# Jordy-VL/multi-modal-early-exit

Measured on AMD Instinct MI355X. Metric: docs_per_sec, higher is better.
Workload: dtype f32 (operands split into 2 x f16, 3 f16 MFMA terms per MAC, f32 accumulate)

## Files before the change

multi-modal-early-exit_amd/csrc/gemm_split.hip:

```cpp
#include <cstdlib>
#include "mmee_common.h"

#include "gemm_split_kernel.h"

namespace mmee {

bool gemm_split_supports(int N, int K) { return N > 0 && K > 0 && N % 256 == 0 && K % 32 == 0; }

void launch_split_ffn_up(const GemmArgs& a, int max_m, int num_cus, hipStream_t s);

void launch_gemm_split(const GemmArgs& a_in, int epi, int max_m, int num_cus, hipStream_t s) {
    GemmArgs a = a_in;
    a.tile_order = a.N <= 768 ? 1 : 0;
    if (a.probe) a.terms = 3;
    if (a.probe) {
        if (a.out_split && epi == EPI_GELU) { launch_split_one<CfgP, EPI_GELU, true, false, 1>(a, max_m, num_cus, s); return; }
        if (!a.out_split && epi == EPI_RESID) { launch_split_one<CfgP, EPI_RESID, false, false, 1>(a, max_m, num_cus, s); return; }
        if (!a.out_split && epi == EPI_BIAS) { launch_split_one<CfgP, EPI_BIAS, false, false, 1>(a, max_m, num_cus, s); return; }
        if (!a.out_split && epi == EPI_TANH) { launch_split_one<CfgP, EPI_TANH, false, false, 1>(a, max_m, num_cus, s); return; }
    }
    if (a.k_splits > 1 && !a.out_split && epi == EPI_BIAS && a.terms != 1) {
        a.tile_counter = nullptr;
        launch_split_one<CfgP, EPI_BIAS, false, false, 1>(a, max_m, num_cus, s);
        return;
    }
    a.k_splits = 1;
    if (a.terms != 1 && (long)((max_m + 255) / 256) * (a.N / 256) * 2 <= (long)num_cus) {
        a.tile_counter = nullptr;
        if (a.out_split && epi == EPI_GELU) { launch_split_one<CfgP, EPI_GELU, true, false, 1>(a, max_m, num_cus, s); return; }
        if (a.out_split && epi == EPI_BIAS) { launch_split_one<CfgP, EPI_BIAS, true, false, 1>(a, max_m, num_cus, s); return; }
        if (!a.out_split && epi == EPI_RESID) { launch_split_one<CfgP, EPI_RESID, false, false, 1>(a, max_m, num_cus, s); return; }
        if (!a.out_split && epi == EPI_BIAS) { launch_split_one<CfgP, EPI_BIAS, false, false, 1>(a, max_m, num_cus, s); return; }
        if (!a.out_split && epi == EPI_TANH) { launch_split_one<CfgP, EPI_TANH, false, false, 1>(a, max_m, num_cus, s); return; }
        a.tile_counter = a_in.tile_counter;
    }
#ifdef MMEE_DIAG
    static const int order_env = diag_env_int("MMEE_GEMM_ORDER", -1);
    if (order_env == 0 || order_env == 1) a.tile_order = order_env;
    else if (order_env == 2) a.tile_order = a.N <= 768 ? 1 : 0;
    else if (order_env == 3 || order_env == 4) a.tile_order = a.N >= 2304 ? order_env - 1 : a.tile_order;
    static const int forced = diag_env_int("MMEE_SPLIT_CFG", 0);
    const bool use_a = forced == 1;
    if (a.dbg_noload && (forced == 0 || forced == 3)) {
        if (a.out_split && epi == EPI_GELU) launch_split_one<CfgC, EPI_GELU, true, true>(a, max_m, num_cus, s);
        else if (a.out_split) launch_split_one<CfgC, EPI_BIAS, true, true>(a, max_m, num_cus, s);
        else launch_split_one<CfgC, EPI_RESID, false, true>(a, max_m, num_cus, s);
        return;
    }
    if (a.dbg_noload) {
        if (a.out_split) launch_split_one<CfgA, EPI_GELU, true, true>(a, max_m, num_cus, s);
        else if (use_a) launch_split_one<CfgA, EPI_RESID, false, true>(a, max_m, num_cus, s);
        else launch_split_one<CfgB, EPI_RESID, false, true>(a, max_m, num_cus, s);
        return;
    }
    if (forced == 1 || forced == 2) {
        if (a.out_split) {
            if (epi == EPI_GELU && use_a) launch_split_one<CfgA, EPI_GELU, true>(a, max_m, num_cus, s);
            else if (epi == EPI_GELU) launch_split_one<CfgB, EPI_GELU, true>(a, max_m, num_cus, s);
            else if (use_a) launch_split_one<CfgA, EPI_BIAS, true>(a, max_m, num_cus, s);
            else launch_split_one<CfgB, EPI_BIAS, true>(a, max_m, num_cus, s);
            return;
        }
        if (use_a) {
            switch (epi) {
                case EPI_BIAS: launch_split_one<CfgA, EPI_BIAS, false>(a, max_m, num_cus, s); break;
                case EPI_GELU: launch_split_one<CfgA, EPI_GELU, false>(a, max_m, num_cus, s); break;
                case EPI_RESID: launch_split_one<CfgA, EPI_RESID, false>(a, max_m, num_cus, s); break;
                default: launch_split_one<CfgA, EPI_TANH, false>(a, max_m, num_cus, s); break;
            }
            return;
        }
        switch (epi) {
            case EPI_BIAS: launch_split_one<CfgB, EPI_BIAS, false>(a, max_m, num_cus, s); break;
            case EPI_GELU: launch_split_one<CfgB, EPI_GELU, false>(a, max_m, num_cus, s); break;
            case EPI_RESID: launch_split_one<CfgB, EPI_RESID, false>(a, max_m, num_cus, s); break;
            default: launch_split_one<CfgB, EPI_TANH, false>(a, max_m, num_cus, s); break;
        }
        return;
    }
#endif
    if (a.terms == 1) {
        if (a.out_split && epi == EPI_GELU) { launch_split_one<CfgC, EPI_GELU, true, false, 0, 1>(a, max_m, num_cus, s); return; }
        if (a.out_split && epi == EPI_BIAS) { launch_split_one<CfgC, EPI_BIAS, true, false, 0, 1>(a, max_m, num_cus, s); return; }
        if (!a.out_split && epi == EPI_RESID) {
            if (a.role_tag == 3) launch_split_one<CfgC, EPI_RESID, false, false, 3, 1>(a, max_m, num_cus, s);
            else launch_split_one<CfgC, EPI_RESID, false, false, 2, 1>(a, max_m, num_cus, s);
            return;
        }
    }
    if (a.out_split) {
        if (epi == EPI_GELU) launch_split_ffn_up(a, max_m, num_cus, s);
        else launch_split_one<CfgC, EPI_BIAS, true>(a, max_m, num_cus, s);
        return;
    }
    switch (epi) {
        case EPI_BIAS: launch_split_one<CfgC, EPI_BIAS, false>(a, max_m, num_cus, s); break;
        case EPI_GELU: launch_split_one<CfgC, EPI_GELU, false>(a, max_m, num_cus, s); break;
        case EPI_RESID:
            if (a.role_tag == 2) launch_split_one<CfgC, EPI_RESID, false, false, 2>(a, max_m, num_cus, s);
            else if (a.role_tag == 3) launch_split_one<CfgC, EPI_RESID, false, false, 3>(a, max_m, num_cus, s);
            else launch_split_one<CfgC, EPI_RESID, false>(a, max_m, num_cus, s);
            break;
        default: launch_split_one<CfgC, EPI_TANH, false>(a, max_m, num_cus, s); break;
    }
}

__global__ __launch_bounds__(256) void split_rows_kernel(const float* __restrict__ src, char* __restrict__ dst, const int* __restrict__ n_rows_ptr,
                                                         int n_rows_static, int K, float scale, int* __restrict__ err_flag) {
    const int n_rows = n_rows_ptr ? *n_rows_ptr : n_rows_static;
    const int k4 = K / 4;
    const size_t total = (size_t)n_rows * k4;
    float amax = 0.f;
    for (size_t i = (size_t)blockIdx.x * 256 + threadIdx.x; i < total; i += (size_t)gridDim.x * 256) {
        const size_t r = i / k4;
        const int c = (int)(i - r * k4) * 4;
        const f32x4 v = *reinterpret_cast<const f32x4*>(src + r * K + c);
        store_split4(dst + r * (size_t)K * 4, c, v, scale, amax);
    }
    split_flag_overflow(amax, err_flag);
}

void launch_split_rows(const float* src, void* dst, const int* n_rows_ptr, int n_rows_static, int max_rows, int K, float scale, int num_cus,
                       hipStream_t s, int* err_flag) {
    size_t total = (size_t)max_rows * (K / 4);
    size_t blocks = (total + 255) / 256;
    int grid = (int)(blocks < (size_t)num_cus * 16 ? blocks : (size_t)num_cus * 16);
    if (grid < 1) grid = 1;
    hipLaunchKernelGGL(split_rows_kernel, dim3(grid), dim3(256), 0, s, src, reinterpret_cast<char*>(dst), n_rows_ptr, n_rows_static, K, scale, err_flag);
}

__global__ __launch_bounds__(256) void patch_split_kernel(const float* __restrict__ pix, char* __restrict__ dst, int n_patches, int C, int R,
                                                          int P, int G, float scale, int* __restrict__ err_flag) {
    const int K = C * P * P, k4 = K / 4;
    const size_t total = (size_t)n_patches * k4;
    float amax = 0.f;
    for (size_t i = (size_t)blockIdx.x * 256 + threadIdx.x; i < total; i += (size_t)gridDim.x * 256) {
        const size_t r = i / k4;
        const int k = (int)(i - r * k4) * 4;
        const int b = (int)(r / (size_t)(G * G)), pr = (int)(r - (size_t)b * (G * G));
        const int gy = pr / G, gx = pr - gy * G;
        const int c = k / (P * P), rem = k - c * P * P;
        const int py = rem / P, px = rem - py * P;
        const f32x4 v = *reinterpret_cast<const f32x4*>(pix + (((size_t)b * C + c) * R + (size_t)(gy * P + py)) * R + gx * P + px);
        store_split4_quad(dst + r * (size_t)K * 4, k, v, scale, amax, threadIdx.x & 63);
    }
    split_flag_overflow(amax, err_flag);
}

void launch_patch_split(const float* pix, void* dst, int n_docs, int C, int R, int P, float scale, int num_cus, hipStream_t s, int* err_flag) {
    const int G = R / P;
    const size_t total = (size_t)n_docs * G * G * (C * P * P / 4);
    size_t blocks = (total + 255) / 256;
    int grid = (int)(blocks < (size_t)num_cus * 16 ? blocks : (size_t)num_cus * 16);
    if (grid < 1) grid = 1;
    hipLaunchKernelGGL(patch_split_kernel, dim3(grid), dim3(256), 0, s, pix, reinterpret_cast<char*>(dst), n_docs * G * G, C, R, P, G, scale, err_flag);
}

__global__ __launch_bounds__(256) void absmax_kernel(const float* __restrict__ src, size_t n, float* __restrict__ out) {
    float m = 0.f;
    for (size_t i = (size_t)blockIdx.x * 256 + threadIdx.x; i < n; i += (size_t)gridDim.x * 256) m = fmaxf(m, fabsf(src[i]));
    m = wave_max(m);
    if ((threadIdx.x & 63) == 0) atomicMax(reinterpret_cast<unsigned*>(out), __float_as_uint(m));
}

void launch_absmax(const float* src, size_t n, float* out_dev, hipStream_t s) {
    (void)hipMemsetAsync(out_dev, 0, sizeof(float), s);
    size_t blocks = (n + 255) / 256;
    int grid = (int)(blocks < 1024 ? blocks : 1024);
    if (grid < 1) grid = 1;
    hipLaunchKernelGGL(absmax_kernel, dim3(grid), dim3(256), 0, s, src, n, out_dev);
}

}
```

multi-modal-early-exit_amd/csrc/gemm_split_ffn_up.hip:

```cpp
#include "gemm_split_kernel.h"

namespace mmee {

void launch_split_ffn_up(const GemmArgs& a, int max_m, int num_cus, hipStream_t s) {
    launch_split_one<CfgC, EPI_GELU, true>(a, max_m, num_cus, s);
}

}
```

multi-modal-early-exit_amd/csrc/gemm_split_kernel.h:

```cpp
#pragma once
#include <cstdlib>
#include "mmee_common.h"

namespace mmee {


template <int BM_, int BN_, int ROWB_, int NST_, int WM_, int WN_, int WGS_, int MF_ = 32>
struct SplitCfg {
    static constexpr int BM = BM_, BN = BN_, ROWB = ROWB_, NST = NST_, WM = WM_, WN = WN_, WGS = WGS_;
    static constexpr int MF = MF_;
    static_assert(MF == 32 || (MF == 16 && ROWB == 128), "the 16x16x32 MFMA consumes one 128-byte row (k = 32) per step");
    static constexpr int NW = WM * WN, THREADS = NW * 64;
    static constexpr int KSTAGE = ROWB / 4;
    static constexpr int PROWS = 1024 / ROWB;
    static constexpr int PA = BM / PROWS / NW, PW = BN / PROWS / NW;
    static constexpr int PP = PA + PW;
    static constexpr int A_BYTES = BM * ROWB, STAGE_BYTES = (BM + BN) * ROWB, LOOP_BYTES = NST * STAGE_BYTES;
    static constexpr int EPI_BYTES = NW * 32 * 64 * 4;
    static_assert(BM == WM * 64 && BN == WN * 64, "one 64x64 sub-tile per wave");
    static_assert(PA * PROWS * NW == BM && PW * PROWS * NW == BN && PA >= 1 && PW >= 1, "DMA pieces must tile the stage");
    static_assert(EPI_BYTES <= LOOP_BYTES, "epilogue staging must fit in the stage ring");
    static_assert(NST >= 2 && NST <= 4, "ring depth");
    static_assert(THREADS <= 1024, "a workgroup is at most 16 waves");
    static_assert(WGS * (LOOP_BYTES + 16) <= 160 * 1024, "LDS budget of a CU (160 KiB) for WGS workgroups");
    static_assert(WGS * NW <= 32, "wave slots of a CU");
};
using CfgA = SplitCfg<128, 256, 64, 3, 2, 4, 2>;
using CfgB = SplitCfg<256, 256, 128, 2, 4, 4, 1>;
using CfgC = SplitCfg<256, 256, 128, 2, 4, 4, 1, 16>;
using CfgP = SplitCfg<128, 128, 128, 3, 2, 2, 1, 16>;


__device__ __forceinline__ void dma_piece(unsigned voff, unsigned long long base, unsigned lds_addr) {
    unsigned keep;
    asm volatile("s_mov_b32 %0, m0\n\ts_mov_b32 m0, %2\n\ts_nop 0\n\tglobal_load_lds_dwordx4 %1, %3\n\ts_mov_b32 m0, %0"
                 : "=&s"(keep)
                 : "v"(voff), "s"(lds_addr), "s"(base)
                 : "memory");
}

template <int EPI, bool OUT_SPLIT, int WN>
__device__ __forceinline__ void split_store_tile(const GemmArgs& g, float* smem, f32x16 (&acc)[2][2], int m0, int n0, int M,
                                                 int wave, int lane) {
    const int wr = wave / WN, wc = wave % WN;
    const int l31 = lane & 31, hh = lane >> 5;
    float* stg = smem + wave * (32 * 64);
    const int c4 = (lane & 15) * 4;
    const int col = n0 + wc * 64 + c4;
    f32x4 bv = f32x4{0.f, 0.f, 0.f, 0.f};
    if (g.bias) bv = *reinterpret_cast<const f32x4*>(g.bias + col);
    const float sc = (col < g.scale_cols) ? g.scale : 1.0f;
    f32x4 lam = f32x4{1.f, 1.f, 1.f, 1.f};
    if (g.col_scale) lam = *reinterpret_cast<const f32x4*>(g.col_scale + col);
    const float alpha = g.alpha;
    float amax = 0.f;
#pragma unroll
    for (int mi = 0; mi < 2; ++mi) {
#pragma unroll
        for (int ni = 0; ni < 2; ++ni)
#pragma unroll
            for (int e = 0; e < 16; ++e) {
                const int r = (e & 3) + 8 * (e >> 2) + 4 * hh;
                stg[r * 64 + ni * 32 + l31] = acc[mi][ni][e];
            }
        asm volatile("" ::: "memory");
        const int rbase = m0 + wr * 64 + mi * 32 + (lane >> 4);
#pragma unroll 4
        for (int j = 0; j < 8; ++j) {
            const int rl = (lane >> 4) + 4 * j;
            const int row = rbase + 4 * j;
            f32x4 v = *reinterpret_cast<const f32x4*>(stg + rl * 64 + c4);
            if (row < M) {
#pragma unroll
                for (int t = 0; t < 4; t += 2) {
                    f32x2 x = __builtin_elementwise_fma(f32x2{v[t], v[t + 1]}, (f32x2)(alpha), f32x2{bv[t], bv[t + 1]}) * (f32x2)(sc);
                    if (EPI == EPI_GELU) x = gelu_erf2(x);
                    if (EPI == EPI_TANH) { x[0] = tanhf(x[0]); x[1] = tanhf(x[1]); }
                    x = x * f32x2{lam[t], lam[t + 1]};
                    v[t] = x[0];
                    v[t + 1] = x[1];
                }
                if (EPI == EPI_RESID) {
                    const int rs = g.resid_row_src ? g.resid_row_src[row] : row;
                    if (g.resid_split_inv != 0.f) {
                        const f32x4 r = load_split4_sum(g.resid + (size_t)rs * g.ldr, col);
#pragma unroll
                        for (int t = 0; t < 4; t += 2) {
                            const f32x2 y = __builtin_elementwise_fma(f32x2{r[t], r[t + 1]}, (f32x2)(g.resid_split_inv), f32x2{v[t], v[t + 1]});
                            v[t] = y[0];
                            v[t + 1] = y[1];
                        }
                    } else {
                        v += *reinterpret_cast<const f32x4*>(g.resid + (size_t)rs * g.ldr + col);
                    }
                }
                if (!OUT_SPLIT) *reinterpret_cast<f32x4*>(g.C + (size_t)row * g.ldc + col) = v;
            }
            if (OUT_SPLIT) {
                f16x4 hi, lo;
                split_f16x4(row < M ? v : f32x4{0.f, 0.f, 0.f, 0.f}, g.out_scale, hi, lo, amax);
                const int2 h2 = __builtin_bit_cast(int2, hi), l2 = __builtin_bit_cast(int2, lo);
                const bool take_lo = (lane & 2) != 0;
                int4 piece;
                {
                    const int a0 = __builtin_amdgcn_mov_dpp(h2.x, 0x88, 0xf, 0xf, true), a1 = __builtin_amdgcn_mov_dpp(h2.y, 0x88, 0xf, 0xf, true);
                    const int b0 = __builtin_amdgcn_mov_dpp(l2.x, 0x88, 0xf, 0xf, true), b1 = __builtin_amdgcn_mov_dpp(l2.y, 0x88, 0xf, 0xf, true);
                    const int c0 = __builtin_amdgcn_mov_dpp(h2.x, 0xDD, 0xf, 0xf, true), c1 = __builtin_amdgcn_mov_dpp(h2.y, 0xDD, 0xf, 0xf, true);
                    const int d0 = __builtin_amdgcn_mov_dpp(l2.x, 0xDD, 0xf, 0xf, true), d1 = __builtin_amdgcn_mov_dpp(l2.y, 0xDD, 0xf, 0xf, true);
                    piece.x = take_lo ? b0 : a0;
                    piece.y = take_lo ? b1 : a1;
                    piece.z = take_lo ? d0 : c0;
                    piece.w = take_lo ? d1 : c1;
                }
                if (row < M)
                    *reinterpret_cast<int4*>(reinterpret_cast<char*>(g.C) + (size_t)row * g.ldc * 4 + (size_t)(col >> 4) * 64 + (lane & 3) * 16) = piece;
            }
        }
    }
    if (OUT_SPLIT) split_flag_overflow(amax, g.err_flag);
}

template <int EPI, bool OUT_SPLIT, int WN, int RB>
__device__ __forceinline__ void split_store_tile16(const GemmArgs& g, float* smem, f32x4 (&acc)[4][4], int m0, int n0, int M,
                                                   int wave, int lane, const f32x4 bv, const f32x4 lam, const size_t c_shift = 0) {
    const int wr = wave / WN, wc = wave % WN;
    const int l15 = lane & 15, gq = lane >> 4;
    float* stg = smem + wave * (RB * 64);
    const int c4 = (lane & 15) * 4;
    const int col = n0 + wc * 64 + c4;
    const float sc = (col < g.scale_cols) ? g.scale : 1.0f;
    const float s_out = OUT_SPLIT ? g.out_scale : 1.0f;
    constexpr bool ACT = EPI == EPI_GELU || EPI == EPI_TANH;
    const bool sc_p2 = (__float_as_uint(sc) & 0x007fffffu) == 0u;
    const float fold = ACT ? 1.0f : s_out * (sc_p2 ? sc : 1.0f);
    const float post = ACT ? sc : (sc_p2 ? 1.0f : sc);
    const bool need_post = __builtin_amdgcn_readfirstlane((int)__float_as_uint(post)) != 0x3f800000;
    const bool need_lam = g.col_scale != nullptr;
    const float alpha_e = g.alpha * fold;
    const f32x4 be = bv * fold;
    const float gelu_c0 = __builtin_log2f(s_out) - 1.0f, gelu_hs = 0.5f * s_out;
    float amax = 0.f;
#pragma unroll
    for (int half = 0; half < 64 / RB; ++half) {
#pragma unroll
        for (int m2 = 0; m2 < RB / 16; ++m2)
#pragma unroll
            for (int ni = 0; ni < 4; ++ni)
#pragma unroll
                for (int e = 0; e < 4; ++e) {
                    const int r = 16 * m2 + 4 * gq + e;
                    stg[r * 64 + ((ni * 16 + l15) ^ (16 * (gq & 1)))] = acc[(RB / 16) * half + m2][ni][e];
                }
        asm volatile("" ::: "memory");
        const int rbase = m0 + wr * 64 + half * RB + (lane >> 4);
#pragma unroll
        for (int j = 0; j < RB / 4; ++j) {
            const int rl = (lane >> 4) + 4 * j;
            const int row = rbase + 4 * j;
            f32x4 v = *reinterpret_cast<const f32x4*>(stg + rl * 64 + (c4 ^ (16 * ((rl >> 2) & 1))));
#pragma unroll
            for (int t = 0; t < 4; t += 2) {
                f32x2 x = __builtin_elementwise_fma(f32x2{v[t], v[t + 1]}, (f32x2)(alpha_e), f32x2{be[t], be[t + 1]});
                if (need_post) x = x * (f32x2)(post);
                if (EPI == EPI_GELU) x = gelu_scaled2(x, gelu_c0, gelu_hs);
                if (EPI == EPI_TANH) { x[0] = tanhf(x[0]) * s_out; x[1] = tanhf(x[1]) * s_out; }
                if (need_lam) x = x * f32x2{lam[t], lam[t + 1]};
                v[t] = x[0];
                v[t + 1] = x[1];
            }
            if (row < M) {
                if (EPI == EPI_RESID) {
                    const int rs = g.resid_row_src ? g.resid_row_src[row] : row;
                    if (g.resid_split_inv != 0.f) {
                        const f32x4 r = load_split4_sum(g.resid + (size_t)rs * g.ldr, col);
#pragma unroll
                        for (int t = 0; t < 4; t += 2) {
                            const f32x2 y = __builtin_elementwise_fma(f32x2{r[t], r[t + 1]}, (f32x2)(g.resid_split_inv), f32x2{v[t], v[t + 1]});
                            v[t] = y[0];
                            v[t + 1] = y[1];
                        }
                    } else {
                        v += *reinterpret_cast<const f32x4*>(g.resid + (size_t)rs * g.ldr + col);
                    }
                }
                if (!OUT_SPLIT) *reinterpret_cast<f32x4*>(g.C + c_shift + (size_t)row * g.ldc + col) = v;
            }
            if (OUT_SPLIT) {
                int2 h2, l2;
                {
                    unsigned h01, h23, l01, l23;
                    split_pair(v[0], v[1], h01, l01, amax);
                    split_pair(v[2], v[3], h23, l23, amax);
                    h2.x = (int)h01; h2.y = (int)h23; l2.x = (int)l01; l2.y = (int)l23;
                }
                const bool take_lo = (lane & 2) != 0;
                int4 piece;
                {
                    const int a0 = __builtin_amdgcn_mov_dpp(h2.x, 0x88, 0xf, 0xf, true), a1 = __builtin_amdgcn_mov_dpp(h2.y, 0x88, 0xf, 0xf, true);
                    const int b0 = __builtin_amdgcn_mov_dpp(l2.x, 0x88, 0xf, 0xf, true), b1 = __builtin_amdgcn_mov_dpp(l2.y, 0x88, 0xf, 0xf, true);
                    const int c0 = __builtin_amdgcn_mov_dpp(h2.x, 0xDD, 0xf, 0xf, true), c1 = __builtin_amdgcn_mov_dpp(h2.y, 0xDD, 0xf, 0xf, true);
                    const int d0 = __builtin_amdgcn_mov_dpp(l2.x, 0xDD, 0xf, 0xf, true), d1 = __builtin_amdgcn_mov_dpp(l2.y, 0xDD, 0xf, 0xf, true);
                    piece.x = take_lo ? b0 : a0;
                    piece.y = take_lo ? b1 : a1;
                    piece.z = take_lo ? d0 : c0;
                    piece.w = take_lo ? d1 : c1;
                }
                if (row < M)
                    *reinterpret_cast<int4*>(reinterpret_cast<char*>(g.C) + (size_t)row * g.ldc * 4 + (size_t)(col >> 4) * 64 + (lane & 3) * 16) = piece;
            }
        }
        asm volatile("" ::: "memory");
    }
    if (OUT_SPLIT) split_flag_overflow(amax, g.err_flag);
}

template <typename Cfg, int EPI, bool OUT_SPLIT, bool DIAG = false, int TAG = 0, int TERMS = 3>
__global__ __launch_bounds__(Cfg::THREADS, 4) void gemm_split_kernel(const GemmArgs g) {
    constexpr int BM = Cfg::BM, BN = Cfg::BN, ROWB = Cfg::ROWB, NST = Cfg::NST, WN = Cfg::WN, PA = Cfg::PA, PW = Cfg::PW;
    constexpr int STAGE_BYTES = Cfg::STAGE_BYTES, A_BYTES = Cfg::A_BYTES;
    const int dbg = DIAG ? g.dbg_noload : 0;
    extern __shared__ __attribute__((aligned(16))) float smem[];
    const int M = g.m_ptr ? *g.m_ptr : g.m_static;
    const int tiles_m = (M + BM - 1) / BM;
    const int tiles_n = g.N / BN;
    constexpr bool KSPLIT = TAG == 1;
    const int ksp = KSPLIT && g.k_splits > 1 ? g.k_splits : 1;
    const int n_tiles = tiles_m * tiles_n * ksp;
    const int nk = g.K / Cfg::KSTAGE / ksp;
    int ks_pop = 0;
    const int tid = threadIdx.x;
    const int lane = tid & 63, wave = __builtin_amdgcn_readfirstlane(tid >> 6);
    const int wr = wave / WN, wc = wave % WN;
    const int l31 = lane & 31, hh = lane >> 5;

    unsigned long long clk0 = 0, rt0 = 0;
    if (DIAG && g.clk_probe) { clk0 = __builtin_amdgcn_s_memtime(); rt0 = __builtin_amdgcn_s_memrealtime(); }
    constexpr int GM = 8;
    int* q_slot = reinterpret_cast<int*>(reinterpret_cast<char*>(smem) + Cfg::LOOP_BYTES);
    const int n_groups = (tiles_m + GM - 1) / GM;
    const int my_xcd = g.tile_counter ? (int)(__builtin_amdgcn_s_getreg((3 << 11) | (0 << 6) | 20) & 7u) : 0;
    int q_try = 0;
    int tile = blockIdx.x;

    const unsigned lds0 = (unsigned)(size_t)(__attribute__((address_space(3))) float*)smem;
    constexpr int CPR = ROWB / 16;
    const int p_row = lane / CPR, p_chunk = lane % CPR;
    const int swz_even = ROWB == 64 ? ((p_row >> 2) & 3) : ((p_row >> 1) & 7);
    const unsigned chunk_even = 16u * (unsigned)(p_chunk ^ swz_even);
    const unsigned chunk_odd = ROWB == 64 ? chunk_even : 16u * (unsigned)(p_chunk ^ ((swz_even + 4) & 7));
    const unsigned rswz = ROWB == 64 ? (unsigned)((l31 >> 2) & 3) : (unsigned)((l31 >> 1) & 7);
    const unsigned a_row = (unsigned)(wr * 64 + l31) * ROWB;
    const unsigned w_row = (unsigned)A_BYTES + (unsigned)(wc * 64 + l31) * ROWB;
    const int l15 = lane & 15, lq = lane >> 4;
    const unsigned swz16 = (unsigned)((l15 >> 1) & 7);
    const unsigned c16_hi = 16u * (((unsigned)(lq & 1) + 4u * (unsigned)(lq >> 1)) ^ swz16);
    const unsigned c16_lo = 16u * (((unsigned)(lq & 1) + 4u * (unsigned)(lq >> 1) + 2u) ^ swz16);
    const unsigned a_row16 = (unsigned)(wr * 64 + l15) * ROWB;
    const unsigned w_row16 = (unsigned)A_BYTES + (unsigned)(wc * 64 + l15) * ROWB;
    const char* sbytes = reinterpret_cast<const char*>(smem);

    constexpr bool HANDOVER = Cfg::MF == 16 && NST == 2 && Cfg::NW * 4096 <= STAGE_BYTES;

    auto pop = [&](int& tm, int& tn) __attribute__((always_inline)) -> bool {
        if (g.tile_counter) {
            while (q_try < 8) {
                const int q = (my_xcd + q_try) & 7;
                if (tid == 0) *q_slot = atomicAdd(g.tile_counter + 16 * q, 1);
                __syncthreads();
                const int j = *q_slot;
                __syncthreads();
                if (g.tile_order >= 2) {
                    const int gq = q < n_groups ? (n_groups - q + 7) / 8 : 0;
                    if (g.tile_order == 2) {
                        constexpr int CW = 4;
                        const int nfull = tiles_n / CW, per_cb = gq * GM * CW;
                        int cb, jj, w;
                        if (per_cb > 0 && j < nfull * per_cb) { cb = j / per_cb; jj = j - cb * per_cb; w = CW; }
                        else { cb = nfull; jj = j - nfull * per_cb; w = tiles_n - CW * nfull; }
                        if (w > 0 && jj < gq * GM * w) {
                            const int gl2 = jj / (GM * w), r2 = jj - gl2 * GM * w;
                            tn = cb * CW + r2 / GM;
                            tm = (q + 8 * gl2) * GM + (r2 - (r2 / GM) * GM);
                            if (tm < tiles_m) return true;
                            continue;
                        }
                    } else {
                        const int per_q = gq * GM * tiles_n;
                        if (j < per_q) {
                            const int pl = j / tiles_n;
                            tn = j - pl * tiles_n;
                            tm = (q + 8 * (pl / GM)) * GM + (pl - (pl / GM) * GM);
                            if (tm < tiles_m) return true;
                            continue;
                        }
                    }
                    ++q_try;
                    continue;
                }
                const int per_group = GM * tiles_n;
                const int gl = j / per_group, r = j - gl * per_group;
                const int grp = q + 8 * gl;
                if (grp < n_groups) {
                    if (g.tile_order == 1) {
                        const int mi = r / tiles_n;
                        tn = r - mi * tiles_n;
                        tm = grp * GM + mi;
                    } else {
                        tn = r / GM;
                        tm = grp * GM + (r - tn * GM);
                    }
                    if (tm < tiles_m) return true;
                    continue;
                }
                ++q_try;
            }
            return false;
        }
        if (tile >= n_tiles) return false;
        int t2 = tile;
        if (KSPLIT) { t2 = tile / ksp; ks_pop = tile - t2 * ksp; }
        tm = t2 / tiles_n;
        tn = t2 - tm * tiles_n;
        tile += gridDim.x;
        return true;
    };

    struct TileCtx {
        int m0, n0;
        int kt0;
        unsigned a_voff[PA], w_voff[PW];
        unsigned long long a_base, w_base;
    };
    auto setup = [&](int tm, int tn, TileCtx& t) __attribute__((always_inline)) {
        t.m0 = __builtin_amdgcn_readfirstlane(tm * BM);
        t.n0 = __builtin_amdgcn_readfirstlane(tn * BN);
        t.kt0 = KSPLIT ? __builtin_amdgcn_readfirstlane(ks_pop * nk) : 0;
        int first = g.row_src ? g.row_src[t.m0] : t.m0;
        if (DIAG && (dbg & 16)) first = 0;
#pragma unroll
        for (int j = 0; j < PA; ++j) {
            const int piece = wave + Cfg::NW * j;
            int ra = t.m0 + Cfg::PROWS * piece + p_row;
            ra = ra < M ? ra : M - 1;
            if (DIAG && (dbg & 16)) ra = Cfg::PROWS * piece + p_row;
            const int sa = g.row_src ? g.row_src[ra] : ra;
            t.a_voff[j] = (unsigned)(sa - first) * (unsigned)g.lda * 4u + ((piece & 1) ? chunk_odd : chunk_even);
        }
#pragma unroll
        for (int j = 0; j < PW; ++j) {
            const int piece = wave + Cfg::NW * j;
            t.w_voff[j] = (unsigned)(Cfg::PROWS * piece + p_row) * (unsigned)g.K * 4u + ((piece & 1) ? chunk_odd : chunk_even);
        }
        const unsigned long long a_base_v = (unsigned long long)(size_t)g.A + (unsigned long long)first * (unsigned)g.lda * 4ull;
        const unsigned long long w_base_v = (unsigned long long)(size_t)g.W + (unsigned long long)t.n0 * (unsigned)g.K * 4ull;
        t.a_base = ((unsigned long long)(unsigned)__builtin_amdgcn_readfirstlane((int)(a_base_v >> 32)) << 32) |
                   (unsigned)__builtin_amdgcn_readfirstlane((int)(a_base_v & 0xffffffffu));
        t.w_base = ((unsigned long long)(unsigned)__builtin_amdgcn_readfirstlane((int)(w_base_v >> 32)) << 32) |
                   (unsigned)__builtin_amdgcn_readfirstlane((int)(w_base_v & 0xffffffffu));
    };
    auto issue = [&](const TileCtx& t, int kt, int buf) __attribute__((always_inline)) {
        const unsigned long long koff = (unsigned long long)(kt + (KSPLIT ? t.kt0 : 0)) * (unsigned)ROWB;
        const unsigned dst = lds0 + (unsigned)buf * STAGE_BYTES + (unsigned)wave * 1024u;
#pragma unroll
        for (int j = 0; j < PA; ++j) dma_piece(t.a_voff[j], t.a_base + koff, dst + (unsigned)(Cfg::NW * j) * 1024u);
#pragma unroll
        for (int j = 0; j < PW; ++j) dma_piece(t.w_voff[j], t.w_base + koff, dst + A_BYTES + (unsigned)(Cfg::NW * j) * 1024u);
    };

    TileCtx cur;
    int buf0 = 0;
    {
        int tm, tn;
        if (!pop(tm, tn)) return;
        setup(tm, tn, cur);
    }
    issue(cur, 0, buf0);
    if (NST >= 3 && nk > 1) issue(cur, 1, 1);
    if (NST >= 4 && nk > 2) issue(cur, 2, 2);
    for (;;) {
        const int m0 = cur.m0, n0 = cur.n0;
        const size_t c_shift = KSPLIT && ksp > 1 ? (size_t)(cur.kt0 / nk) * g.split_stride : 0;
        f32x16 acc[2][2];
        f32x4 acc16[4][4];
        if constexpr (Cfg::MF == 32) {
#pragma unroll
            for (int i = 0; i < 2; ++i)
#pragma unroll
                for (int j = 0; j < 2; ++j)
#pragma unroll
                    for (int e = 0; e < 16; ++e) acc[i][j][e] = 0.f;
        } else {
#pragma unroll
            for (int i = 0; i < 4; ++i)
#pragma unroll
                for (int j = 0; j < 4; ++j) acc16[i][j] = f32x4{0.f, 0.f, 0.f, 0.f};
        }

        int buf = buf0, bufn = (buf0 + NST - 1) % NST;
        for (int kt = 0; kt < nk; ++kt) {
            if ((dbg & 6) == 6) {
            } else if (dbg & 2) {
                asm volatile("s_waitcnt vmcnt(0)" ::: "memory");
            } else if (dbg & 4) {
                asm volatile("s_barrier" ::: "memory");
            } else if (NST == 4 && kt + 2 < nk) {
                static_assert(NST != 4 || Cfg::PP == 8, "vmcnt immediate: two stages' pieces per wave");
                asm volatile("s_waitcnt vmcnt(16)\n\ts_barrier" ::: "memory");
            } else if (NST >= 3 && kt + 1 < nk) {
                static_assert(Cfg::PP == 3 || Cfg::PP == 4 || Cfg::PP == 8, "vmcnt immediate: one stage's pieces per wave");
                if (Cfg::PP == 3) asm volatile("s_waitcnt vmcnt(3)\n\ts_barrier" ::: "memory");
                else if (Cfg::PP == 4) asm volatile("s_waitcnt vmcnt(4)\n\ts_barrier" ::: "memory");
                else asm volatile("s_waitcnt vmcnt(8)\n\ts_barrier" ::: "memory");
            } else {
                asm volatile("s_waitcnt vmcnt(0)\n\ts_barrier" ::: "memory");
            }
            if (kt + NST - 1 < nk && !(dbg & 1)) issue(cur, kt + NST - 1, bufn);
            const char* sb = sbytes + buf * STAGE_BYTES;
            if constexpr (Cfg::MF == 16) {
                f16x8 ah[4], al[4];
#pragma unroll
                for (int i = 0; i < 4; ++i) {
                    ah[i] = *reinterpret_cast<const f16x8*>(sb + a_row16 + c16_hi + i * 16 * ROWB);
                    al[i] = *reinterpret_cast<const f16x8*>(sb + a_row16 + c16_lo + i * 16 * ROWB);
                }
#pragma unroll
                for (int j = 0; j < 4; ++j) {
                    const f16x8 wh = *reinterpret_cast<const f16x8*>(sb + w_row16 + c16_hi + j * 16 * ROWB);
                    const f16x8 wl = *reinterpret_cast<const f16x8*>(sb + w_row16 + c16_lo + j * 16 * ROWB);
                    if (TERMS == 3) {
#pragma unroll
                        for (int i = 0; i < 4; ++i) acc16[i][j] = __builtin_amdgcn_mfma_f32_16x16x32_f16(al[i], wh, acc16[i][j], 0, 0, 0);
#pragma unroll
                        for (int i = 0; i < 4; ++i) acc16[i][j] = __builtin_amdgcn_mfma_f32_16x16x32_f16(ah[i], wl, acc16[i][j], 0, 0, 0);
                    }
#pragma unroll
                    for (int i = 0; i < 4; ++i) acc16[i][j] = __builtin_amdgcn_mfma_f32_16x16x32_f16(ah[i], wh, acc16[i][j], 0, 0, 0);
                }
            } else
#pragma unroll
            for (int ks = 0; ks < ROWB / 64; ++ks) {
                const unsigned c_hi = 16u * (((unsigned)(4 * ks) + (unsigned)hh) ^ rswz);
                const unsigned c_lo = 16u * (((unsigned)(4 * ks + 2) + (unsigned)hh) ^ rswz);
                f16x8 ah[2], al[2], wh[2], wl[2];
#pragma unroll
                for (int i = 0; i < 2; ++i) {
                    ah[i] = *reinterpret_cast<const f16x8*>(sb + a_row + c_hi + i * 32 * ROWB);
                    al[i] = *reinterpret_cast<const f16x8*>(sb + a_row + c_lo + i * 32 * ROWB);
                    wh[i] = *reinterpret_cast<const f16x8*>(sb + w_row + c_hi + i * 32 * ROWB);
                    wl[i] = *reinterpret_cast<const f16x8*>(sb + w_row + c_lo + i * 32 * ROWB);
                }
#pragma unroll
                for (int i = 0; i < 2; ++i)
#pragma unroll
                    for (int j = 0; j < 2; ++j) {
                        acc[i][j] = __builtin_amdgcn_mfma_f32_32x32x16_f16(al[i], wh[j], acc[i][j], 0, 0, 0);
                        acc[i][j] = __builtin_amdgcn_mfma_f32_32x32x16_f16(ah[i], wl[j], acc[i][j], 0, 0, 0);
                        acc[i][j] = __builtin_amdgcn_mfma_f32_32x32x16_f16(ah[i], wh[j], acc[i][j], 0, 0, 0);
                    }
            }
            buf = buf == NST - 1 ? 0 : buf + 1;
            bufn = bufn == NST - 1 ? 0 : bufn + 1;
        }
        __syncthreads();
        f32x4 bv = f32x4{0.f, 0.f, 0.f, 0.f}, lam = f32x4{1.f, 1.f, 1.f, 1.f};
        if constexpr (Cfg::MF == 16) {
            const int col = n0 + wc * 64 + (lane & 15) * 4;
            if (g.bias) bv = *reinterpret_cast<const f32x4*>(g.bias + col);
            if (g.col_scale) lam = *reinterpret_cast<const f32x4*>(g.col_scale + col);
            asm volatile("s_waitcnt vmcnt(0)" : "+v"(bv), "+v"(lam) :: "memory");
        }
        TileCtx nxt;
        bool have;
        {
            int tm, tn;
            have = pop(tm, tn);
            if (have) setup(tm, tn, nxt);
        }
        const int last_slot = (buf0 + nk - 1) % NST;
        const int nbuf0 = HANDOVER ? (last_slot ^ 1) : 0;
        if (HANDOVER && have) issue(nxt, 0, nbuf0);
        if (!(dbg & 8)) {
            if constexpr (Cfg::MF == 16) {
                if constexpr (HANDOVER)
                    split_store_tile16<EPI, OUT_SPLIT, WN, 16>(g, smem + last_slot * (STAGE_BYTES / 4), acc16, m0, n0, M, wave, lane, bv, lam);
                else
                    split_store_tile16<EPI, OUT_SPLIT, WN, 32>(g, smem, acc16, m0, n0, M, wave, lane, bv, lam, c_shift);
            } else {
                split_store_tile<EPI, OUT_SPLIT, WN>(g, smem, acc, m0, n0, M, wave, lane);
            }
        }
        __syncthreads();
        if (!have) break;
        cur = nxt;
        buf0 = nbuf0;
        if (!HANDOVER) {
            issue(cur, 0, 0);
            if (NST >= 3 && nk > 1) issue(cur, 1, 1);
            if (NST >= 4 && nk > 2) issue(cur, 2, 2);
        }
    }
    if (DIAG && g.clk_probe && threadIdx.x == 0) {
        g.clk_probe[2 * blockIdx.x] = __builtin_amdgcn_s_memtime() - clk0;
        g.clk_probe[2 * blockIdx.x + 1] = __builtin_amdgcn_s_memrealtime() - rt0;
    }
}

template <typename Cfg, int EPI, bool OUT_SPLIT, bool DIAG = false, int TAG = 0, int TERMS = 3>
static void launch_split_one(const GemmArgs& a, int max_m, int num_cus, hipStream_t s) {
    const size_t lds = Cfg::LOOP_BYTES + 16;
    (void)ensure_dynamic_lds<&gemm_split_kernel<Cfg, EPI, OUT_SPLIT, DIAG, TAG, TERMS>>("gemm_split_kernel", (int)lds);
    const int tiles = ((max_m + Cfg::BM - 1) / Cfg::BM) * (a.N / Cfg::BN) * (TAG == 1 && a.k_splits > 1 ? a.k_splits : 1);
    int grid = Cfg::WGS * num_cus;
    if (grid > tiles) grid = tiles;
    if (grid < 1) grid = 1;
    hipLaunchKernelGGL((gemm_split_kernel<Cfg, EPI, OUT_SPLIT, DIAG, TAG, TERMS>), dim3(grid), dim3(Cfg::THREADS), lds, s, a);
}

}
```

Baseline: 6982.

## Add phased 256x256 split-f16 GEMM kernel with quadrant-interleaved loads and DMA

Adds a new persistent 256x256-tile GEMM kernel for the three-term split-f16 path. Each K step is split into four quadrant phases that interleave LDS fragment reads, asynchronous global-to-LDS DMA for the next stages, and MFMA bursts, using double-buffered half-tiles. The next tile's prologue loads are issued before the epilogue. Release builds route the bias, tanh, output-split bias and FFN-up GELU GEMMs to the new kernel, while the residual GEMMs stay on the old path. This aims to hide memory latency and raise MFMA utilisation, at the cost of more complex synchronisation and one-CU-wide grids that may underfill small problems.

```diff
diff --git a/multi-modal-early-exit_amd/csrc/gemm_split.hip b/multi-modal-early-exit_amd/csrc/gemm_split.hip
--- a/multi-modal-early-exit_amd/csrc/gemm_split.hip
+++ b/multi-modal-early-exit_amd/csrc/gemm_split.hip
@@ -1,13 +1,13 @@
 #include <cstdlib>
 #include "mmee_common.h"
 
-#include "gemm_split_kernel.h"
+#include "gemm_split_phased.h"
 
 namespace mmee {
 
 bool gemm_split_supports(int N, int K) { return N > 0 && K > 0 && N % 256 == 0 && K % 32 == 0; }
 
-void launch_split_ffn_up(const GemmArgs& a, int max_m, int num_cus, hipStream_t s);
+void launch_split_ffn_up(const GemmArgs& a, int max_m, int num_cus, hipStream_t s, bool phased);
 
 void launch_gemm_split(const GemmArgs& a_in, int epi, int max_m, int num_cus, hipStream_t s) {
     GemmArgs a = a_in;
@@ -88,20 +88,53 @@
             return;
         }
     }
+    static_assert(kPhasedRoles == (1 | 4), "the release routing below is written for this mask");
+#ifdef MMEE_DIAG
+    static const int phased_env = diag_env_int("MMEE_GEMM_PHASED", -1);
+    const int phased = phased_env >= 0 ? phased_env : kPhasedRoles;
+#endif
     if (a.out_split) {
-        if (epi == EPI_GELU) launch_split_ffn_up(a, max_m, num_cus, s);
-        else launch_split_one<CfgC, EPI_BIAS, true>(a, max_m, num_cus, s);
+        if (epi == EPI_GELU) {
+#ifdef MMEE_DIAG
+            launch_split_ffn_up(a, max_m, num_cus, s, (phased & 4) != 0);
+#else
+            launch_split_ffn_up(a, max_m, num_cus, s, true);
+#endif
+            return;
+        }
+#ifdef MMEE_DIAG
+        if (!(phased & 1)) { launch_split_one<CfgC, EPI_BIAS, true>(a, max_m, num_cus, s); return; }
+#endif
+        launch_split_phased<EPI_BIAS, true>(a, max_m, num_cus, s);
         return;
     }
     switch (epi) {
-        case EPI_BIAS: launch_split_one<CfgC, EPI_BIAS, false>(a, max_m, num_cus, s); break;
+        case EPI_BIAS:
+#ifdef MMEE_DIAG
+            if (!(phased & 1)) { launch_split_one<CfgC, EPI_BIAS, false>(a, max_m, num_cus, s); break; }
+#endif
+            launch_split_phased<EPI_BIAS, false>(a, max_m, num_cus, s);
+            break;
         case EPI_GELU: launch_split_one<CfgC, EPI_GELU, false>(a, max_m, num_cus, s); break;
         case EPI_RESID:
+#ifdef MMEE_DIAG
+            if (phased & ((a.role_tag == 3 || (a.role_tag != 2 && a.K > a.N)) ? 8 : 2)) {
+                if (a.role_tag == 2) launch_split_phased<EPI_RESID, false, 2>(a, max_m, num_cus, s);
+                else if (a.role_tag == 3) launch_split_phased<EPI_RESID, false, 3>(a, max_m, num_cus, s);
+                else launch_split_phased<EPI_RESID, false>(a, max_m, num_cus, s);
+                break;
+            }
+#endif
             if (a.role_tag == 2) launch_split_one<CfgC, EPI_RESID, false, false, 2>(a, max_m, num_cus, s);
             else if (a.role_tag == 3) launch_split_one<CfgC, EPI_RESID, false, false, 3>(a, max_m, num_cus, s);
             else launch_split_one<CfgC, EPI_RESID, false>(a, max_m, num_cus, s);
             break;
-        default: launch_split_one<CfgC, EPI_TANH, false>(a, max_m, num_cus, s); break;
+        default:
+#ifdef MMEE_DIAG
+            if (!(phased & 1)) { launch_split_one<CfgC, EPI_TANH, false>(a, max_m, num_cus, s); break; }
+#endif
+            launch_split_phased<EPI_TANH, false>(a, max_m, num_cus, s);
+            break;
     }
 }
 
diff --git a/multi-modal-early-exit_amd/csrc/gemm_split_ffn_up.hip b/multi-modal-early-exit_amd/csrc/gemm_split_ffn_up.hip
--- a/multi-modal-early-exit_amd/csrc/gemm_split_ffn_up.hip
+++ b/multi-modal-early-exit_amd/csrc/gemm_split_ffn_up.hip
@@ -1,9 +1,13 @@
-#include "gemm_split_kernel.h"
+#include "gemm_split_phased.h"
 
 namespace mmee {
 
-void launch_split_ffn_up(const GemmArgs& a, int max_m, int num_cus, hipStream_t s) {
-    launch_split_one<CfgC, EPI_GELU, true>(a, max_m, num_cus, s);
+void launch_split_ffn_up(const GemmArgs& a, int max_m, int num_cus, hipStream_t s, bool phased) {
+#ifdef MMEE_DIAG
+    if (!phased) { launch_split_one<CfgC, EPI_GELU, true>(a, max_m, num_cus, s); return; }
+#endif
+    (void)phased;
+    launch_split_phased<EPI_GELU, true>(a, max_m, num_cus, s);
 }
 
 }
diff --git a/multi-modal-early-exit_amd/csrc/gemm_split_kernel.h b/multi-modal-early-exit_amd/csrc/gemm_split_kernel.h
--- a/multi-modal-early-exit_amd/csrc/gemm_split_kernel.h
+++ b/multi-modal-early-exit_amd/csrc/gemm_split_kernel.h
@@ -122,7 +122,8 @@
 
 template <int EPI, bool OUT_SPLIT, int WN, int RB>
 __device__ __forceinline__ void split_store_tile16(const GemmArgs& g, float* smem, f32x4 (&acc)[4][4], int m0, int n0, int M,
-                                                   int wave, int lane, const f32x4 bv, const f32x4 lam, const size_t c_shift = 0) {
+                                                   int wave, int lane, const f32x4 bv, const f32x4 lam, const size_t c_shift = 0,
+                                                   const int row_off = 0) {
     const int wr = wave / WN, wc = wave % WN;
     const int l15 = lane & 15, gq = lane >> 4;
     float* stg = smem + wave * (RB * 64);
@@ -152,7 +153,7 @@
                     stg[r * 64 + ((ni * 16 + l15) ^ (16 * (gq & 1)))] = acc[(RB / 16) * half + m2][ni][e];
                 }
         asm volatile("" ::: "memory");
-        const int rbase = m0 + wr * 64 + half * RB + (lane >> 4);
+        const int rbase = m0 + row_off + wr * 64 + half * RB + (lane >> 4);
 #pragma unroll
         for (int j = 0; j < RB / 4; ++j) {
             const int rl = (lane >> 4) + 4 * j;
diff --git a/multi-modal-early-exit_amd/csrc/gemm_split_phased.h b/multi-modal-early-exit_amd/csrc/gemm_split_phased.h
--- /dev/null
+++ b/multi-modal-early-exit_amd/csrc/gemm_split_phased.h
@@ -0,0 +1,258 @@
+#pragma once
+#include "gemm_split_kernel.h"
+
+namespace mmee {
+
+template <int BM_, int BN_, int MF_>
+struct PhasedCfg {
+    static_assert(BM_ == 256 && BN_ == 256 && MF_ == 16, "the phased loop exists for the 256 x 256 tile on v_mfma_f32_16x16x32_f16");
+    static constexpr int BM = BM_, BN = BN_, MF = MF_, ROWB = 128, KSTAGE = 32, WM = 2, WN = 4, NW = 8, THREADS = 512, WGS = 1;
+    static constexpr int HALF_BYTES = 128 * ROWB, BUF_BYTES = 4 * HALF_BYTES, LOOP_BYTES = 2 * BUF_BYTES;
+    static constexpr int EPI_OFF = 6 * HALF_BYTES;
+    static_assert(NW * 4096 == 2 * HALF_BYTES, "4 KB of staging per wave");
+};
+using CfgH = PhasedCfg<256, 256, 16>;
+constexpr int kPhasedRoles = 1 | 4;
+
+template <typename Cfg, int EPI, bool OUT_SPLIT, bool DIAG = false, int TAG = 0, int TERMS = 3>
+__global__ __launch_bounds__(Cfg::THREADS, 2) void gemm_split_phased_kernel(const GemmArgs g) {
+    static_assert(!DIAG && TERMS == 3 && TAG != 1, "release form, three terms, no split-K");
+    constexpr int BM = Cfg::BM, BN = Cfg::BN, ROWB = Cfg::ROWB, NW = Cfg::NW;
+    constexpr unsigned HALF = Cfg::HALF_BYTES, BUFB = Cfg::BUF_BYTES;
+    extern __shared__ __attribute__((aligned(16))) float smem[];
+    const int M = g.m_ptr ? *g.m_ptr : g.m_static;
+    const int tiles_m = (M + BM - 1) / BM;
+    const int tiles_n = g.N / BN;
+    const int n_tiles = tiles_m * tiles_n;
+    const int nk = g.K / Cfg::KSTAGE;
+    const int tid = threadIdx.x;
+    const int lane = tid & 63, wave = __builtin_amdgcn_readfirstlane(tid >> 6);
+    const int wr = wave >> 2, wc = wave & 3;
+
+    constexpr int GM = 8;
+    int* q_slot = reinterpret_cast<int*>(reinterpret_cast<char*>(smem) + Cfg::LOOP_BYTES);
+    const int n_groups = (tiles_m + GM - 1) / GM;
+    const int my_xcd = g.tile_counter ? (int)(__builtin_amdgcn_s_getreg((3 << 11) | (0 << 6) | 20) & 7u) : 0;
+    int q_try = 0;
+    int tile = blockIdx.x;
+
+    const unsigned lds0 = (unsigned)(size_t)(__attribute__((address_space(3))) float*)smem;
+    const int p_row = lane >> 3, p_chunk = lane & 7;
+    const unsigned chunk = 16u * (unsigned)(p_chunk ^ ((((p_row >> 1) & 7) + 4 * (wave & 1)) & 7));
+    const int l15 = lane & 15, lq = lane >> 4;
+    const unsigned swz16 = (unsigned)((l15 >> 1) & 7);
+    const unsigned rd_hi = (unsigned)l15 * ROWB + 16u * (((unsigned)(lq & 1) + 4u * (unsigned)(lq >> 1)) ^ swz16);
+    const unsigned rd_lo = (unsigned)l15 * ROWB + 16u * (((unsigned)(lq & 1) + 4u * (unsigned)(lq >> 1) + 2u) ^ swz16);
+    const unsigned w_rd = (unsigned)(wc * 32) * ROWB, a_rd = HALF + (unsigned)(wr * 64) * ROWB;
+    const char* sbytes = reinterpret_cast<const char*>(smem);
+
+    auto pop = [&](int& tm, int& tn) __attribute__((always_inline)) -> bool {
+        if (g.tile_counter) {
+            while (q_try < 8) {
+                const int q = (my_xcd + q_try) & 7;
+                if (tid == 0) *q_slot = atomicAdd(g.tile_counter + 16 * q, 1);
+                __syncthreads();
+                const int j = *q_slot;
+                __syncthreads();
+                const int per_group = GM * tiles_n;
+                const int gl = j / per_group, r = j - gl * per_group;
+                const int grp = q + 8 * gl;
+                if (grp < n_groups) {
+                    if (g.tile_order == 1) {
+                        const int mi = r / tiles_n;
+                        tn = r - mi * tiles_n;
+                        tm = grp * GM + mi;
+                    } else {
+                        tn = r / GM;
+                        tm = grp * GM + (r - tn * GM);
+                    }
+                    if (tm < tiles_m) return true;
+                    continue;
+                }
+                ++q_try;
+            }
+            return false;
+        }
+        if (tile >= n_tiles) return false;
+        tm = tile / tiles_n;
+        tn = tile - tm * tiles_n;
+        tile += gridDim.x;
+        return true;
+    };
+
+    struct TileCtx {
+        int m0, n0;
+        unsigned a_voff[2][2], w_voff[2][2];
+        unsigned long long a_base, w_base;
+    };
+    auto setup = [&](int tm, int tn, TileCtx& t) __attribute__((always_inline)) {
+        t.m0 = __builtin_amdgcn_readfirstlane(tm * BM);
+        t.n0 = __builtin_amdgcn_readfirstlane(tn * BN);
+        const int first = g.row_src ? g.row_src[t.m0] : t.m0;
+#pragma unroll
+        for (int h = 0; h < 2; ++h)
+#pragma unroll
+            for (int j = 0; j < 2; ++j) {
+                const int lr = 8 * (wave + NW * j) + p_row;
+                int ra = t.m0 + (lr >> 6) * 128 + h * 64 + (lr & 63);
+                ra = ra < M ? ra : M - 1;
+                const int sa = g.row_src ? g.row_src[ra] : ra;
+                t.a_voff[h][j] = (unsigned)(sa - first) * (unsigned)g.lda * 4u + chunk;
+                t.w_voff[h][j] = (unsigned)((lr >> 5) * 64 + h * 32 + (lr & 31)) * (unsigned)g.K * 4u + chunk;
+            }
+        const unsigned long long a_base_v = (unsigned long long)(size_t)g.A + (unsigned long long)first * (unsigned)g.lda * 4ull;
+        const unsigned long long w_base_v = (unsigned long long)(size_t)g.W + (unsigned long long)t.n0 * (unsigned)g.K * 4ull;
+        t.a_base = ((unsigned long long)(unsigned)__builtin_amdgcn_readfirstlane((int)(a_base_v >> 32)) << 32) |
+                   (unsigned)__builtin_amdgcn_readfirstlane((int)(a_base_v & 0xffffffffu));
+        t.w_base = ((unsigned long long)(unsigned)__builtin_amdgcn_readfirstlane((int)(w_base_v >> 32)) << 32) |
+                   (unsigned)__builtin_amdgcn_readfirstlane((int)(w_base_v & 0xffffffffu));
+    };
+    auto issue = [&](const TileCtx& t, int kt, int slot, unsigned boff) __attribute__((always_inline)) {
+        const unsigned long long koff = (unsigned long long)kt * (unsigned)ROWB;
+        const unsigned dst = lds0 + boff + (unsigned)slot * HALF + (unsigned)wave * 1024u;
+        const int h = slot >> 1;
+        if (slot & 1) {
+            dma_piece(t.a_voff[h][0], t.a_base + koff, dst);
+            dma_piece(t.a_voff[h][1], t.a_base + koff, dst + NW * 1024u);
+        } else {
+            dma_piece(t.w_voff[h][0], t.w_base + koff, dst);
+            dma_piece(t.w_voff[h][1], t.w_base + koff, dst + NW * 1024u);
+        }
+    };
+    auto issue_first = [&](const TileCtx& t) __attribute__((always_inline)) {
+#pragma unroll
+        for (int s = 0; s < 4; ++s) issue(t, 0, s, 0u);
+        if (nk > 1) {
+            issue(t, 1, 0, BUFB);
+            issue(t, 1, 1, BUFB);
+        }
+    };
+    auto quadrant = [&](f32x4 (&c)[4][4], int jb, const f16x8 (&ah)[4], const f16x8 (&al)[4], const f16x8 (&wh)[2], const f16x8 (&wl)[2])
+                        __attribute__((always_inline)) {
+        __builtin_amdgcn_s_setprio(1);
+#pragma unroll
+        for (int j = 0; j < 2; ++j)
+#pragma unroll
+            for (int i = 0; i < 4; ++i) c[i][jb + j] = __builtin_amdgcn_mfma_f32_16x16x32_f16(al[i], wh[j], c[i][jb + j], 0, 0, 0);
+#pragma unroll
+        for (int j = 0; j < 2; ++j)
+#pragma unroll
+            for (int i = 0; i < 4; ++i) c[i][jb + j] = __builtin_amdgcn_mfma_f32_16x16x32_f16(ah[i], wl[j], c[i][jb + j], 0, 0, 0);
+#pragma unroll
+        for (int j = 0; j < 2; ++j)
+#pragma unroll
+            for (int i = 0; i < 4; ++i) c[i][jb + j] = __builtin_amdgcn_mfma_f32_16x16x32_f16(ah[i], wh[j], c[i][jb + j], 0, 0, 0);
+        __builtin_amdgcn_s_setprio(0);
+    };
+
+    TileCtx cur;
+    {
+        int tm, tn;
+        if (!pop(tm, tn)) return;
+        setup(tm, tn, cur);
+    }
+    issue_first(cur);
+    for (;;) {
+        const int m0 = cur.m0, n0 = cur.n0;
+        f32x4 acc[2][4][4];
+#pragma unroll
+        for (int h = 0; h < 2; ++h)
+#pragma unroll
+            for (int i = 0; i < 4; ++i)
+#pragma unroll
+                for (int j = 0; j < 4; ++j) acc[h][i][j] = f32x4{0.f, 0.f, 0.f, 0.f};
+
+        __builtin_amdgcn_s_barrier();
+        if (nk > 1) {
+            issue(cur, 1, 2, BUFB);
+            asm volatile("s_waitcnt vmcnt(6)" ::: "memory");
+        } else {
+            asm volatile("s_waitcnt vmcnt(0)" ::: "memory");
+        }
+        __builtin_amdgcn_s_barrier();
+
+        unsigned boff = 0;
+        for (int kt = 0; kt < nk; ++kt) {
+            const char* sb = sbytes + boff;
+            f16x8 ah[4], al[4], w0h[2], w0l[2], w1h[2], w1l[2];
+#pragma unroll
+            for (int j = 0; j < 2; ++j) {
+                w0h[j] = *reinterpret_cast<const f16x8*>(sb + w_rd + rd_hi + j * 16 * ROWB);
+                w0l[j] = *reinterpret_cast<const f16x8*>(sb + w_rd + rd_lo + j * 16 * ROWB);
+            }
+            __builtin_amdgcn_sched_barrier(0);
+#pragma unroll
+            for (int i = 0; i < 4; ++i) {
+                ah[i] = *reinterpret_cast<const f16x8*>(sb + a_rd + rd_hi + i * 16 * ROWB);
+                al[i] = *reinterpret_cast<const f16x8*>(sb + a_rd + rd_lo + i * 16 * ROWB);
+            }
+            __builtin_amdgcn_sched_barrier(0);
+            if (kt + 1 < nk) issue(cur, kt + 1, 3, boff ^ BUFB);
+            asm volatile("s_waitcnt lgkmcnt(8)" ::: "memory");
+            __builtin_amdgcn_s_barrier();
+            asm volatile("s_waitcnt lgkmcnt(0)" ::: "memory");
+            quadrant(acc[0], 0, ah, al, w0h, w0l);
+#pragma unroll
+            for (int j = 0; j < 2; ++j) {
+                w1h[j] = *reinterpret_cast<const f16x8*>(sb + w_rd + 2 * HALF + rd_hi + j * 16 * ROWB);
+                w1l[j] = *reinterpret_cast<const f16x8*>(sb + w_rd + 2 * HALF + rd_lo + j * 16 * ROWB);
+            }
+            if (kt + 2 < nk) issue(cur, kt + 2, 0, boff);
+            __builtin_amdgcn_s_barrier();
+            asm volatile("s_waitcnt lgkmcnt(0)" ::: "memory");
+            quadrant(acc[0], 2, ah, al, w1h, w1l);
+#pragma unroll
+            for (int i = 0; i < 4; ++i) {
+                ah[i] = *reinterpret_cast<const f16x8*>(sb + a_rd + 2 * HALF + rd_hi + i * 16 * ROWB);
+                al[i] = *reinterpret_cast<const f16x8*>(sb + a_rd + 2 * HALF + rd_lo + i * 16 * ROWB);
+            }
+            if (kt + 2 < nk) issue(cur, kt + 2, 1, boff);
+            __builtin_amdgcn_s_barrier();
+            asm volatile("s_waitcnt lgkmcnt(0)" ::: "memory");
+            quadrant(acc[1], 2, ah, al, w1h, w1l);
+            if (kt + 2 < nk) {
+                issue(cur, kt + 2, 2, boff);
+                asm volatile("s_waitcnt vmcnt(6)" ::: "memory");
+            } else if (kt + 1 < nk) {
+                asm volatile("s_waitcnt vmcnt(0)" ::: "memory");
+            }
+            __builtin_amdgcn_s_barrier();
+            quadrant(acc[1], 0, ah, al, w0h, w0l);
+            boff ^= BUFB;
+        }
+        f32x4 bv = f32x4{0.f, 0.f, 0.f, 0.f}, lam = f32x4{1.f, 1.f, 1.f, 1.f};
+        {
+            const int col = n0 + wc * 64 + (lane & 15) * 4;
+            if (g.bias) bv = *reinterpret_cast<const f32x4*>(g.bias + col);
+            if (g.col_scale) lam = *reinterpret_cast<const f32x4*>(g.col_scale + col);
+            asm volatile("s_waitcnt vmcnt(0)" : "+v"(bv), "+v"(lam) :: "memory");
+        }
+        TileCtx nxt;
+        bool have;
+        {
+            int tm, tn;
+            have = pop(tm, tn);
+            if (have) setup(tm, tn, nxt);
+        }
+        if (have) issue_first(nxt);
+        float* stg = smem + Cfg::EPI_OFF / 4;
+#pragma unroll
+        for (int h = 0; h < 2; ++h)
+            split_store_tile16<EPI, OUT_SPLIT, Cfg::WN, 16>(g, stg, acc[h], m0, n0, M, wave, lane, bv, lam, 0, wr * 64 + h * 64);
+        if (!have) break;
+        cur = nxt;
+    }
+}
+
+template <int EPI, bool OUT_SPLIT, int TAG = 0>
+static void launch_split_phased(const GemmArgs& a, int max_m, int num_cus, hipStream_t s) {
+    const size_t lds = CfgH::LOOP_BYTES + 16;
+    (void)ensure_dynamic_lds<&gemm_split_phased_kernel<CfgH, EPI, OUT_SPLIT, false, TAG, 3>>("gemm_split_phased_kernel", (int)lds);
+    const int tiles = ((max_m + CfgH::BM - 1) / CfgH::BM) * (a.N / CfgH::BN);
+    int grid = num_cus;
+    if (grid > tiles) grid = tiles;
+    if (grid < 1) grid = 1;
+    hipLaunchKernelGGL((gemm_split_phased_kernel<CfgH, EPI, OUT_SPLIT, false, TAG, 3>), dim3(grid), dim3(CfgH::THREADS), lds, s, a);
+}
+
+}
```

New measurement: 7028 (median of 6 runs). No clear change (+0.7%).
